# benrobaglia/D2D-PPO

Measured on AMD Instinct MI355X. Metric: env-steps/sec (agents×envs) + PPO updates/sec, 64 agents × 8 ch, 1/2/4/8 GPU, higher is better.
Workload: dtype u8

## Files before the change

### d2d-ppo_amd/csrc/common.h

```cpp
#pragma once
#include <hip/hip_runtime.h>
#include <stdint.h>

#include "d2d_hip.h"

namespace d2d {

constexpr int kWave = 64;

enum : uint32_t { kStreamFlip = 0, kStreamArrival = 1, kStreamAction = 2, kPerEnv = 0xFFFFFFFFu };

struct u32x4 {
  uint32_t x, y, z, w;
};

__device__ __forceinline__ u32x4 philox(uint32_t c0, uint32_t c1, uint32_t c2, uint32_t c3, uint64_t seed) {
  uint32_t k0 = (uint32_t)seed, k1 = (uint32_t)(seed >> 32);
#pragma unroll
  for (int r = 0; r < 10; ++r) {
    if (r) {
      k0 += 0x9E3779B9u;
      k1 += 0xBB67AE85u;
    }
    const uint64_t p0 = (uint64_t)0xD2511F53u * c0;
    const uint64_t p1 = (uint64_t)0xCD9E8D57u * c2;
    uint32_t n0, n2;
    asm("v_bitop3_b32 %0, %1, %2, %3 bitop3:0x96" : "=v"(n0) : "v"((uint32_t)(p1 >> 32)), "v"(c1), "s"(k0));
    asm("v_bitop3_b32 %0, %1, %2, %3 bitop3:0x96" : "=v"(n2) : "v"((uint32_t)(p0 >> 32)), "v"(c3), "s"(k1));
    c0 = n0;
    c1 = (uint32_t)p1;
    c2 = n2;
    c3 = (uint32_t)p0;
  }
  return {c0, c1, c2, c3};
}

__device__ __forceinline__ uint32_t pick(const u32x4& r, int i) {
  return i == 0 ? r.x : (i == 1 ? r.y : (i == 2 ? r.z : r.w));
}

__device__ __forceinline__ uint32_t poisson_lookup(uint32_t r, const uint32_t* __restrict__ t) {
  uint32_t x = 0;
  for (;;) {
    const uint4 q = *reinterpret_cast<const uint4*>(t + x);
    const uint32_t n = (uint32_t)(r > q.x) + (uint32_t)(r > q.y) + (uint32_t)(r > q.z) + (uint32_t)(r > q.w);
    x += n;
    if (n < 4u) return x;
  }
}

}

void d2d_set_error(const char* fmt, ...);

#define D2D_CHECK_HIP(expr)                                                    \
  do {                                                                         \
    hipError_t _e = (expr);                                                    \
    if (_e != hipSuccess) {                                                    \
      d2d_set_error("%s: %s", #expr, hipGetErrorString(_e));                   \
      return D2D_EHIP;                                                         \
    }                                                                          \
  } while (0)

inline int obs_format_args(int32_t format, const uint32_t* sgn_in, int32_t obs_dim, const void* obs, const float*& f32,
                           const uint8_t*& rec, const uint32_t*& sgn) {
  f32 = nullptr; rec = nullptr; sgn = nullptr;
  if (format == D2D_OBS_F32) { f32 = static_cast<const float*>(obs); return D2D_OK; }
  if (format != D2D_OBS_U8) { d2d_set_error("unknown obs_format %d", format); return D2D_EINVAL; }
  if (!sgn_in) { d2d_set_error("obs_format D2D_OBS_U8 needs obs_signed"); return D2D_EINVAL; }
  if (reinterpret_cast<uintptr_t>(obs) & 15) { d2d_set_error("the obs record must be 16-byte aligned"); return D2D_EINVAL; }
  (void)obs_dim;
  rec = static_cast<const uint8_t*>(obs); sgn = sgn_in;
  return D2D_OK;
}
```

### d2d-ppo_amd/csrc/env_kernels.hip

```cpp
#include <atomic>
#include <cmath>
#include <cstdarg>
#include <cstdio>
#include <cstring>

#include "common.h"
#include "policy_split.h"

namespace d2d {

constexpr int kBlock = 256;
constexpr int kCombWavesPerEu = 7;
constexpr int kCombRecBlock = 256;
constexpr int kMaxAgents = 1024;

struct EnvArgs {
  int E, N, C, D, F, S, state_stride, seg, reset, cnt_words;
  uint32_t flags;
  uint32_t rng_step;
  uint64_t env_base, seed;
  const d2d_agent_entry* agents;
  const uint64_t* flip_thr;
  const uint32_t* pois_cdf;
  uint32_t* buf;
  void* chan;
  uint32_t* recv;
  uint32_t* disc;
  uint32_t* selq;
  uint32_t* seln;
  const void* actions;
  const void* flips;
  const uint8_t* arrivals;
  float* obs;
  uint8_t* rec;
  int rec_bytes;
  float* state;
  uint16_t* state_b;
  int64_t state_b_ld;
  int32_t* reward;
  void* ack;
  uint8_t* success;
  const int32_t* gather;
  const uint32_t* rng_off;
  uint64_t draw[kMaxAgents / 64];
};

template <int DW>
struct Row {
  uint32_t w[DW];
};

template <int DW>
__device__ __forceinline__ void load_row(Row<DW>& r, const uint32_t* p) {
  if constexpr (DW == 4) {
    const uint4 v = *reinterpret_cast<const uint4*>(p);
    r.w[0] = v.x; r.w[1] = v.y; r.w[2] = v.z; r.w[3] = v.w;
  } else if constexpr (DW == 2) {
    const uint2 v = *reinterpret_cast<const uint2*>(p);
    r.w[0] = v.x; r.w[1] = v.y;
  } else if constexpr (DW == 8) {
    const uint4 v0 = reinterpret_cast<const uint4*>(p)[0];
    const uint4 v1 = reinterpret_cast<const uint4*>(p)[1];
    r.w[0] = v0.x; r.w[1] = v0.y; r.w[2] = v0.z; r.w[3] = v0.w;
    r.w[4] = v1.x; r.w[5] = v1.y; r.w[6] = v1.z; r.w[7] = v1.w;
  } else {
#pragma unroll
    for (int i = 0; i < DW; ++i) r.w[i] = p[i];
  }
}

template <int DW>
__device__ __forceinline__ void store_row(const Row<DW>& r, uint32_t* p) {
  if constexpr (DW == 4) {
    *reinterpret_cast<uint4*>(p) = make_uint4(r.w[0], r.w[1], r.w[2], r.w[3]);
  } else if constexpr (DW == 2) {
    *reinterpret_cast<uint2*>(p) = make_uint2(r.w[0], r.w[1]);
  } else if constexpr (DW == 8) {
    reinterpret_cast<uint4*>(p)[0] = make_uint4(r.w[0], r.w[1], r.w[2], r.w[3]);
    reinterpret_cast<uint4*>(p)[1] = make_uint4(r.w[4], r.w[5], r.w[6], r.w[7]);
  } else {
#pragma unroll
    for (int i = 0; i < DW; ++i) p[i] = r.w[i];
  }
}

template <int DW>
__device__ __forceinline__ bool row_any(const Row<DW>& r) {
// ... 66 lines not shown

template <typename T>
__device__ __forceinline__ void st_stream(T* p, const T& v, bool nt) {
  if (nt)
    __builtin_nontemporal_store(v, p);
  else
    *p = v;
}

__device__ __forceinline__ void flush_contig(float* __restrict__ dst, const float* src, int count, bool nt) {
  const bool vec = ((reinterpret_cast<uintptr_t>(dst) & 15) == 0) && ((count & 3) == 0);
  if (vec) {
    float4* d4 = reinterpret_cast<float4*>(dst);
    const float4* s4 = reinterpret_cast<const float4*>(src);
    for (int i = threadIdx.x; i < (count >> 2); i += blockDim.x) {
      const float4 v = s4[i];
      if (nt) {
        __builtin_nontemporal_store(v.x, &d4[i].x);
        __builtin_nontemporal_store(v.y, &d4[i].y);
        __builtin_nontemporal_store(v.z, &d4[i].z);
        __builtin_nontemporal_store(v.w, &d4[i].w);
      } else {
        d4[i] = v;
      }
    }
  } else {
    for (int i = threadIdx.x; i < count; i += blockDim.x) st_stream(dst + i, src[i], nt);
  }
}

__device__ __forceinline__ void flush_rows(float* __restrict__ dst, int stride, const float* src, int rows, int S,
                                           bool nt) {
  if ((S & 3) == 0 && (stride & 3) == 0 && ((reinterpret_cast<uintptr_t>(dst) & 15) == 0)) {
    const int q = S >> 2;
    for (int i = threadIdx.x; i < rows * q; i += blockDim.x) {
      const int r = i / q, j = i - r * q;
      float4* d4 = reinterpret_cast<float4*>(dst + (size_t)r * stride) + j;
      const float4 v = reinterpret_cast<const float4*>(src + r * S)[j];
      if (nt) {
        __builtin_nontemporal_store(v.x, &d4->x);
        __builtin_nontemporal_store(v.y, &d4->y);
        __builtin_nontemporal_store(v.z, &d4->z);
        __builtin_nontemporal_store(v.w, &d4->w);
      } else {
        *d4 = v;
      }
    }
  } else {
    for (int i = threadIdx.x; i < rows * S; i += blockDim.x) {
      const int r = i / S, j = i - r * S;
      st_stream(dst + (size_t)r * stride + j, src[r * S + j], nt);
    }
  }
}

struct Lane {
  int env, k, local_env, envs_per_block, lane;
  bool active;
  uint64_t segmask;
};

template <bool LARGE>
__device__ __forceinline__ Lane lane_geometry(const EnvArgs& a, int bidx = blockIdx.x) {
  Lane L;
  L.lane = threadIdx.x & (kWave - 1);
  if (LARGE) {
    L.env = bidx;
    L.k = threadIdx.x;
    L.local_env = 0;
    L.envs_per_block = 1;
    L.segmask = ~0ull;
  } else {
    L.local_env = threadIdx.x / a.seg;
    L.k = threadIdx.x - L.local_env * a.seg;
    L.envs_per_block = blockDim.x / a.seg;
    L.env = bidx * L.envs_per_block + L.local_env;
    const int seg_base = L.lane & ~(a.seg - 1);
    L.segmask = (a.seg == kWave) ? ~0ull : (((1ull << a.seg) - 1ull) << seg_base);
  }
  L.active = (L.k < a.N) && (L.env < a.E);
  return L;
}

template <bool LARGE>
__device__ __forceinline__ int env_count(bool v, const Lane& L, int* lds_acc) {
  const int part = __popcll(__ballot(v) & L.segmask);
  if (!LARGE) return part;
  if (L.lane == 0) atomicAdd(lds_acc, part);
  __syncthreads();
  const int tot = *lds_acc;
  return tot;
}

__device__ __forceinline__ void wave_lds_sync() {
  __builtin_amdgcn_s_waitcnt(0xC07F);
  __builtin_amdgcn_wave_barrier();
  asm volatile("" ::: "memory");
}

__device__ __forceinline__ void wave_flush(float* __restrict__ dst, const float* src, int count, bool nt) {
  const int lane = threadIdx.x & (kWave - 1);
  if (((reinterpret_cast<uintptr_t>(dst) & 15) == 0) && ((reinterpret_cast<uintptr_t>(src) & 15) == 0) &&
      ((count & 3) == 0)) {
    float4* d4 = reinterpret_cast<float4*>(dst);
    const float4* s4 = reinterpret_cast<const float4*>(src);
    for (int i = lane; i < (count >> 2); i += kWave) {
      const float4 v = s4[i];
      if (nt) {
        __builtin_nontemporal_store(v.x, &d4[i].x);
        __builtin_nontemporal_store(v.y, &d4[i].y);
        __builtin_nontemporal_store(v.z, &d4[i].z);
        __builtin_nontemporal_store(v.w, &d4[i].w);
      } else {
        d4[i] = v;
      }
    }
  } else {
    for (int i = lane; i < count; i += kWave) st_stream(dst + i, src[i], nt);
  }
}

__device__ __forceinline__ void flush_bf16(uint16_t* __restrict__ dst, const float* src, int S, int first, int stride,
                                           bool nt) {
  const int q8 = (S + 7) >> 3;
  for (int q = first; q < q8; q += stride) {
    uint32_t w[4];
#pragma unroll
    for (int p = 0; p < 4; ++p) {
      const int j = 8 * q + 2 * p;
      const uint32_t lo = j < S ? __float_as_uint(src[j]) >> 16 : 0u;
      const uint32_t hi = j + 1 < S ? __float_as_uint(src[j + 1]) & 0xFFFF0000u : 0u;
      w[p] = lo | hi;
    }
    st_rec(reinterpret_cast<uint4*>(dst) + q, w[0], w[1], w[2], w[3], nt);
  }
}

template <typename MaskT, int DW, bool LARGE, int CT, bool RESET, bool PACKED = false>
__device__ __forceinline__ void comb_step(const EnvArgs a, float* lds, int bidx, uint4* lrec, int lstride, int lenv0) {
  const Lane L = lane_geometry<LARGE>(a, bidx);
  const int N = a.N, F = a.F;
  const int C = CT ? CT : a.C;
  const int wave = threadIdx.x >> 6;
  const int nwaves = blockDim.x >> 6;
  int* cnt = reinterpret_cast<int*>(lds);
  const int slot = (kWave * F + 3) & ~3;
  float* lds_obs = lds + a.cnt_words + wave * slot;
  const int epw = LARGE ? 1 : kWave / a.seg;
  float* lds_state = LARGE ? lds + a.cnt_words + nwaves * slot
                           : lds + a.cnt_words + nwaves * slot + wave * ((epw * a.S + 3) & ~3);
  const size_t row = (size_t)L.env * N + L.k;
  const uint64_t genv = a.env_base + (uint64_t)L.env;
  const uint32_t cmask = (C >= 32) ? 0xFFFFFFFFu : ((1u << C) - 1u);
  constexpr int kMaskShift = 32 - 8 * (int)sizeof(MaskT);
  constexpr uint32_t kRowKeep = sizeof(MaskT) >= 4 ? 0u : ((1u << (kMaskShift & 31)) - 1u);

  Row<DW> b;
#pragma unroll
  for (int i = 0; i < DW; ++i) b.w[i] = 0;
  uint32_t h_pre = cmask, act = 0, rc = 0, dc = 0;
  d2d_agent_entry ag{};
  if (L.active) {
    ag = a.agents[L.k];
    if (!RESET) {
      load_row<DW>(b, a.buf + row * DW);
      act = (uint32_t)reinterpret_cast<const MaskT*>(a.actions)[row] & cmask;
      if constexpr (PACKED) {
        h_pre = (b.w[DW - 1] >> kMaskShift) & cmask;
        b.w[DW - 1] &= kRowKeep;
        const uint32_t cw = a.recv[row];
        rc = cw & 0xFFFFu;
        dc = cw >> 16;
      } else {
        h_pre = (uint32_t)reinterpret_cast<const MaskT*>(a.chan)[row] & cmask;
        rc = a.recv[row];
        dc = a.disc[row];
      }
    }
  }
  if (LARGE) {
    if (threadIdx.x < 80) cnt[threadIdx.x] = 0;
    __syncthreads();
  }

  uint32_t ack_one = cmask, ack_zero = 0, h_new = h_pre;
  bool succ = false;
  int nsucc = 0;
  if (!RESET) {
    ack_one = 0;
    const uint32_t att = row_any<DW>(b) ? act : 0u;
    const uint32_t good = att & h_pre;
    auto count_channel = [&](int c) {
      const uint64_t m = __ballot((att >> c) & 1u) & L.segmask;
      const uint64_t g = __ballot((good >> c) & 1u) & L.segmask;
      if (!LARGE) {
        const int n = __popcll(m);
        ack_zero |= (uint32_t)(n == 0) << c;
        ack_one |= (uint32_t)(n == 1 && g != 0) << c;
      } else if (L.lane == 0) {
        atomicAdd(&cnt[c], __popcll(m));
        atomicAdd(&cnt[32 + c], __popcll(g));
      }
    };
    if constexpr (CT != 0) {
#pragma unroll
      for (int c = 0; c < CT; ++c) count_channel(c);
    } else {
      for (int c = 0; c < C; ++c) count_channel(c);
    }
    if (LARGE) {
      __syncthreads();
      for (int c = 0; c < C; ++c) {
        const int n = cnt[c];
        ack_zero |= (uint32_t)(n == 0) << c;
        ack_one |= (uint32_t)(n == 1 && cnt[32 + c] == 1) << c;
      }
    }
    succ = L.active && ((good & ack_one) != 0);
    nsucc = env_count<LARGE>(succ, L, cnt + 64);
    if (succ) row_remove_first<DW>(b);
    dc += row_expire_shift<DW>(b);
    uint32_t f = 0;
    if (L.active) {
      if (a.flips) {
        f = (uint32_t)reinterpret_cast<const MaskT*>(a.flips)[row];
      } else {
        const uint64_t* thr = a.flip_thr + (size_t)L.k * C;
        auto flip_block = [&](int blk) {
          const u32x4 r = philox((uint32_t)genv, (uint32_t)L.k, rng_of(a), (kStreamFlip << 24) | (uint32_t)blk, a.seed);
#pragma unroll
          for (int i = 0; i < 4; ++i) {
            const int c = blk * 4 + i;
            if (c < C) f |= (uint32_t)((uint64_t)pick(r, i) < thr[c]) << c;
          }
        };
        if constexpr (CT != 0) {
#pragma unroll
          for (int blk = 0; blk < (CT + 3) / 4; ++blk) flip_block(blk);
        } else {
          for (int blk = 0; blk * 4 < C; ++blk) flip_block(blk);
        }
      }
    }
    h_new = (h_pre ^ f) & cmask;
  }
  const bool drew = L.active && (LARGE ? draws_now(a, L.k) : ((a.draw[0] >> L.k) & 1ull));
  if (drew) {
    const uint32_t x = arrival_value(a, ag, row, L.k, genv);
    row_set<DW>(b, (int)ag.deadline - 1, x);
    rc = (RESET ? 0u : rc) + x;
  } else if (RESET) {
    rc = 0;
  }
  if (RESET) dc = 0;
  if (L.active) {
    if constexpr (PACKED) {
      Row<DW> o = b;
      o.w[DW - 1] |= h_new << kMaskShift;
      store_row<DW>(o, a.buf + row * DW);
      a.recv[row] = rc | (dc << 16);
    } else {
      store_row<DW>(b, a.buf + row * DW);
      reinterpret_cast<MaskT*>(a.chan)[row] = (MaskT)h_new;
      a.recv[row] = rc;
      a.disc[row] = dc;
    }
    if (!RESET) {
      if (a.success) a.success[row] = succ ? 1 : 0;
      if (L.k == 0) {
        if (a.reward) a.reward[L.env] = nsucc;
        if (a.ack) {
          int8_t* ak = reinterpret_cast<int8_t*>(a.ack) + (size_t)L.env * C;
          for (int c = 0; c < C; ++c) ak[c] = ((ack_one >> c) & 1) ? 1 : (((ack_zero >> c) & 1) ? 0 : -1);
        }
      }
    }
  }
  const int wave_env0 = LARGE ? bidx : (bidx * L.envs_per_block + wave * epw);
  const int wave_nenv = LARGE ? 1 : max(0, min(epw, a.E - wave_env0));
  if (a.obs) {
    if (L.active) {
      const int lrow = LARGE ? (L.k - wave * kWave) : ((L.local_env - wave * epw) * N + L.k);
      float* o = lds_obs + lrow * F;
      const int w = ag.obs_width;
#pragma unroll
      for (int j = 0; j < DW * 4; ++j)
        if (j < w) o[j] = row_byte<DW>(b, j);
      auto obs_channel = [&](int c) {
        o[w + c] = (float)((h_pre >> c) & 1u);
        o[w + C + c] = ((ack_one >> c) & 1u) ? 1.f : (((ack_zero >> c) & 1u) ? 0.f : -1.f);
      };
      if constexpr (CT != 0) {
#pragma unroll
        for (int c = 0; c < CT; ++c) obs_channel(c);
      } else {
        for (int c = 0; c < C; ++c) obs_channel(c);
      }
      for (int j = w + 2 * C; j < F; ++j) o[j] = 0.f;
    }
    wave_lds_sync();
    if (LARGE) {
      const int k0 = wave * kWave;
      const int nrows = max(0, min(kWave, N - k0));
      if (nrows > 0) wave_flush(a.obs + ((size_t)bidx * N + k0) * F, lds_obs, nrows * F, a.flags & 1u);
    } else if (wave_nenv > 0) {
      wave_flush(a.obs + (size_t)wave_env0 * N * F, lds_obs, wave_nenv * N * F, a.flags & 1u);
    }
  }
  if (a.rec && L.active) {
    const int w = ag.obs_width;
    const uint32_t ack_neg = ~(ack_one | ack_zero) & cmask;
    auto tail_byte = [&](int p) -> uint32_t {
      const int m = p - w;
      if (m < C) return (h_pre >> m) & 1u;
      const int c = m - C;
      if (c < C) return ((ack_one >> c) & 1u) | (((ack_neg >> c) & 1u) * 0xFFu);
      return p == F ? 1u : 0u;
    };
    uint4* dst = reinterpret_cast<uint4*>(a.rec + row * (size_t)a.rec_bytes);
    uint32_t v[8];
    bool built = false;
    if constexpr (CT != 0 && 2 * CT <= 16 && 4 * DW <= 16) {
      if (a.rec_bytes == 32) {
        constexpr int NB = CT / 2;
        auto expand4 = [](uint32_t n) { return (n * 0x204081u) & 0x01010101u; };
        uint32_t blk[NB];
#pragma unroll
        for (int u = 0; u < CT / 4; ++u) {
          blk[u] = expand4((h_pre >> (4 * u)) & 0xFu);
          blk[CT / 4 + u] = expand4((ack_one >> (4 * u)) & 0xFu) | expand4((ack_neg >> (4 * u)) & 0xFu) * 0xFFu;
        }
        const int ws = w >> 2, bs = w & 3;
        uint32_t sh[NB + 1];
#pragma unroll
        for (int j = 0; j <= NB; ++j) {
          const uint32_t hi = j < NB ? blk[j] : 0u, lo = j > 0 ? blk[j - 1] : 0u;
          sh[j] = bs == 0 ? hi : __builtin_amdgcn_alignbyte(hi, lo, 4 - bs);
        }
#pragma unroll
        for (int q = 0; q < 8; ++q) {
          uint32_t word = q < DW ? b.w[q < DW ? q : 0] : 0u;
#pragma unroll
          for (int c = 0; c <= 16 / 4; ++c)
            if (q - c >= 0 && q - c <= NB) word |= ws == c ? sh[q - c] : 0u;
          word |= (q == (F >> 2)) ? (1u << (8 * (F & 3))) : 0u;
          v[q] = word;
        }
        const bool nt = a.flags & 1u;
        st_rec(dst, v[0], v[1], v[2], v[3], nt);
        st_rec(dst + 1, v[4], v[5], v[6], v[7], nt);
        if (lrec) {
          uint4* l = lrec + (size_t)L.k * lstride + 2 * (L.env - lenv0);
          l[0] = make_uint4(v[0], v[1], v[2], v[3]);
          l[1] = make_uint4(v[4], v[5], v[6], v[7]);
        }
        built = true;
      }
    }
    if (!built) {
#pragma unroll
    for (int q = 0; q < 8; ++q) {
      uint32_t word = 0;
#pragma unroll
      for (int j = 0; j < 4; ++j) {
        const int p = 4 * q + j;
        const uint32_t bb = p < 4 * DW ? (b.w[(p < 4 * DW ? p : 0) >> 2] >> (8 * (p & 3))) & 0xFFu : 0u;
        word |= (p < w ? bb : tail_byte(p)) << (8 * j);
      }
      v[q] = word;
    }
    dst[0] = make_uint4(v[0], v[1], v[2], v[3]);
    dst[1] = make_uint4(v[4], v[5], v[6], v[7]);
    if (lrec) {
      uint4* l = lrec + (size_t)L.k * lstride + 2 * (L.env - lenv0);
      l[0] = make_uint4(v[0], v[1], v[2], v[3]);
      l[1] = make_uint4(v[4], v[5], v[6], v[7]);
    }
    for (int q32 = 1; q32 < a.rec_bytes / 32; ++q32) {
#pragma unroll
      for (int q = 0; q < 8; ++q) {
        uint32_t word = 0;
#pragma unroll
        for (int j = 0; j < 4; ++j) word |= tail_byte(32 * q32 + 4 * q + j) << (8 * j);
        v[q] = word;
      }
      dst[2 * q32] = make_uint4(v[0], v[1], v[2], v[3]);
      dst[2 * q32 + 1] = make_uint4(v[4], v[5], v[6], v[7]);
    }
    }
  }
  if (a.state || a.state_b) {
    if (L.active) {
      float* st = lds_state + (LARGE ? 0 : (L.local_env - wave * epw) * a.S);
      const int off = ag.state_offset, d = ag.deadline;
#pragma unroll
      for (int j = 0; j < DW * 4; ++j)
        if (j < d) st[off + j] = row_byte<DW>(b, j);
      const int sb = a.S - C * (N + 1);
      for (int c = 0; c < C; ++c) st[sb + L.k * C + c] = (float)((h_new >> c) & 1u);
      if (L.k == 0)
        for (int c = 0; c < C; ++c)
          st[sb + N * C + c] = ((ack_one >> c) & 1u) ? 1.f : (((ack_zero >> c) & 1u) ? 0.f : -1.f);
    }
    if (LARGE) {
      __syncthreads();
      if (a.state) flush_rows(a.state + (size_t)bidx * a.state_stride, a.state_stride, lds_state, 1, a.S, a.flags & 1u);
      if (a.state_b) flush_bf16(a.state_b + (size_t)bidx * a.state_b_ld, lds_state, a.S, threadIdx.x, blockDim.x, a.flags & 1u);
    } else {
      wave_lds_sync();
      for (int r = 0; r < wave_nenv; ++r) {
        if (a.state)
          wave_flush(a.state + (size_t)(wave_env0 + r) * a.state_stride, lds_state + r * a.S, a.S, a.flags & 1u);
        if (a.state_b)
          flush_bf16(a.state_b + (size_t)(wave_env0 + r) * a.state_b_ld, lds_state + r * a.S, a.S, L.lane, kWave,
                     a.flags & 1u);
      }
    }
  }
}

template <typename MaskT, int DW, bool LARGE, int CT, bool RESET, bool PACKED = false>
__global__ __launch_bounds__(kMaxAgents) __attribute__((amdgpu_waves_per_eu(kCombWavesPerEu))) void comb_kernel(EnvArgs a) {
  extern __shared__ __attribute__((aligned(16))) float lds[];
  comb_step<MaskT, DW, LARGE, CT, RESET, PACKED>(a, lds, blockIdx.x, nullptr, 0, 0);
}

template <int DW, bool PACK>
__global__ __launch_bounds__(256) void comb_state_repack_kernel(int64_t n, uint32_t* buf, uint8_t* chan, uint32_t* recv,
                                                                uint32_t* disc, uint32_t* rows, uint32_t* counters) {
  const int64_t i = (int64_t)blockIdx.x * blockDim.x + threadIdx.x;
  if (i >= n) return;
  Row<DW> b;
  if (PACK) {
    load_row<DW>(b, buf + i * DW);
    b.w[DW - 1] = (b.w[DW - 1] & 0x00FFFFFFu) | ((uint32_t)chan[i] << 24);
    store_row<DW>(b, rows + i * DW);
    counters[i] = (recv[i] & 0xFFFFu) | (disc[i] << 16);
  } else {
    load_row<DW>(b, rows + i * DW);
    chan[i] = (uint8_t)(b.w[DW - 1] >> 24);
    b.w[DW - 1] &= 0x00FFFFFFu;
    store_row<DW>(b, buf + i * DW);
    const uint32_t cw = counters[i];
    recv[i] = cw & 0xFFFFu;
    disc[i] = cw >> 16;
  }
}

template <int DW, int HT, int SE, int MODE>
__global__ __launch_bounds__(256, SE <= 32 ? 2 : 1) void comb_policy_fused_kernel(EnvArgs e, MlpArgs p) {
  static_assert(SE % 32 == 0, "the policy runs 16-env tiles in pairs");
  constexpr int LSTR = 2 * SE + 1;
  __shared__ uint4 lrec[64 * LSTR];
  const int env0 = blockIdx.x * SE;
  for (int q = 0; q < SE / 4; ++q)
    comb_step<uint8_t, DW, false, 8, false>(e, nullptr, blockIdx.x * (SE / 4) + q, lrec, LSTR, env0);
  __syncthreads();
  const uint32_t rng = (MODE == kModeSample && p.rng_off) ? p.rng_step + *p.rng_off : p.rng_step;
  const int lane = threadIdx.x & 63, g = lane >> 4, i = lane & 15;
  const int wave = __builtin_amdgcn_readfirstlane(threadIdx.x >> 6);
  for (int k = wave; k < p.N; k += 4) {
    SplitNet<1, HT, true, false> net;
    net.load(p, k, g, i);
    uint32_t sm[1][2];
    record_sign_masks<1>(sm, p.sgn, k, g);
    const uint4* row = lrec + k * LSTR;
    auto tile = [&](int t, f32x4& lg) {
      const uint2 w = reinterpret_cast<const uint2*>(row + 2 * (16 * t + i))[g];
      const uint32_t d[1][2] = {{w.x, w.y}};
      float xc[1][8];
      stage_record_words<1>(xc, d, sm);
      float v;
      net.template tile<true>(xc, lg, v);
    };
    for (int tt = 0; tt < SE / 16; tt += 2) {
      f32x4 lg0, lg1;
      tile(tt, lg0);
      tile(tt + 1, lg1);
      f32x4 lgc;
#pragma unroll
      for (int r = 0; r < 4; ++r) lgc[r] = uf(__builtin_amdgcn_permlane32_swap(fu(lg0[r]), fu(lg1[r]), false, false)[0]);
      const int envc = env0 + tt * 16 + i + (g < 2 ? 0 : 16);
      policy_epilogue<0, false, true, MODE>(p, lgc, 0.f, envc, envc < p.E, k, g, rng);
    }
  }
}

template <int DW, bool LARGE>
__global__ __launch_bounds__(kMaxAgents) void chsel_kernel(EnvArgs a) {
  extern __shared__ __attribute__((aligned(16))) float lds[];
  const Lane L = lane_geometry<LARGE>(a);
  const int N = a.N, C = a.C, F = a.F;
  int* cnt_all = reinterpret_cast<int*>(lds);
  int* cnt = cnt_all + L.local_env * 34;
  float* lds_obs = lds + a.cnt_words;
  float* lds_state = lds_obs + ((L.envs_per_block * N * F + 3) & ~3);
  const size_t row = (size_t)L.env * N + L.k;
  const uint64_t genv = a.env_base + (uint64_t)L.env;
  const uint32_t hmask = (C + 1 >= 32) ? 0xFFFFFFFFu : ((1u << (C + 1)) - 1u);
  uint32_t* chan = reinterpret_cast<uint32_t*>(a.chan);
  const bool env_ok = L.env < a.E;

  Row<DW> b;
#pragma unroll
  for (int i = 0; i < DW; ++i) b.w[i] = 0;
  uint32_t H = hmask, act = 0, rc = 0, dc = 0;
  d2d_agent_entry ag{};
// ... 341 lines not shown
  if (!comb && !single && d->env_kind != D2D_ENV_CHANNEL_SELECTION) { d2d_set_error("unknown env_kind %d", d->env_kind); return D2D_EINVAL; }
  if (single) {
    if (d->n_agents < 1 || d->n_agents > kMaxAgents) { d2d_set_error("n_agents=%d outside [1,%d]", d->n_agents, kMaxAgents); return D2D_EUNSUPPORTED; }
    if (d->n_channels != 1) { d2d_set_error("the single-channel env needs n_channels == 1"); return D2D_EINVAL; }
    if (d->max_deadline < 1 || d->max_deadline > 32) { d2d_set_error("max_deadline=%d outside [1,32]", d->max_deadline); return D2D_EUNSUPPORTED; }
    if (d->n_envs < 0) { d2d_set_error("n_envs < 0"); return D2D_EINVAL; }
    if (d->obs_dim < 2 || d->state_dim != 0 && d->state_stride < d->state_dim) { d2d_set_error("bad obs/state dims"); return D2D_EINVAL; }
    if (!d->agents || !d->flip_thr || !d->arrival_kind_host || !d->period_host || !d->offset_host || !d->gather ||
        !d->poisson_cdf) {
      d2d_set_error("desc tables (incl. the gather map and poisson_cdf) must be non-NULL"); return D2D_EINVAL;
    }
    return D2D_OK;
  }
  if (d->n_agents < 1 || d->n_agents > kMaxAgents) { d2d_set_error("n_agents=%d outside [1,%d]", d->n_agents, kMaxAgents); return D2D_EUNSUPPORTED; }
  if (d->n_channels < 1 || d->n_channels > (comb ? 32 : 31)) { d2d_set_error("n_channels=%d unsupported", d->n_channels); return D2D_EUNSUPPORTED; }
  if (d->max_deadline < 1 || d->max_deadline > 32) { d2d_set_error("max_deadline=%d outside [1,32]", d->max_deadline); return D2D_EUNSUPPORTED; }
  if (d->n_envs < 0) { d2d_set_error("n_envs < 0"); return D2D_EINVAL; }
  const int F = comb ? d->max_deadline + 2 * d->n_channels : d->max_deadline + d->n_channels + 1;
  if (d->obs_dim != F) { d2d_set_error("obs_dim=%d, expected %d", d->obs_dim, F); return D2D_EINVAL; }
  if (d->state_stride < d->state_dim) { d2d_set_error("state_stride < state_dim"); return D2D_EINVAL; }
  if (!d->agents || !d->flip_thr || !d->arrival_kind_host || !d->period_host || !d->offset_host || !d->poisson_cdf) {
    d2d_set_error("desc tables (incl. poisson_cdf) must be non-NULL"); return D2D_EINVAL;
  }
  return D2D_OK;
}

void draw_mask(const d2d_env_desc* d, int t, uint64_t* mask) {
  memset(mask, 0, sizeof(uint64_t) * (kMaxAgents / 64));
  for (int k = 0; k < d->n_agents; ++k) {
    const int kind = d->arrival_kind_host[k];
    bool dr = kind == D2D_ARRIVAL_POISSON;
    if (kind == D2D_ARRIVAL_SCHEDULED_BERNOULLI) dr = std::fmod((double)t, d->period_host[k]) == d->offset_host[k];
    if (dr) mask[k >> 6] |= 1ull << (k & 63);
  }
}

template <typename K>
int set_lds(K kernel, size_t bytes) {
  if (bytes > 163840) { d2d_set_error("LDS requirement %zu B exceeds 160 KiB (N*obs_dim too large)", bytes); return D2D_EUNSUPPORTED; }
  if (bytes > 65536)
    D2D_CHECK_HIP(hipFuncSetAttribute(reinterpret_cast<const void*>(kernel), hipFuncAttributeMaxDynamicSharedMemorySize, (int)bytes));
  return D2D_OK;
}

size_t lds_need(const EnvArgs& a, int block, int kind) {
  const bool large = a.N > kWave;
  const bool stage = a.obs || a.state || a.state_b;
  const bool comb = kind == D2D_ENV_COMBINATORIAL;
  if (kind == D2D_ENV_SINGLE) {
    const int epb = large ? 1 : block / a.seg;
    return sizeof(float) * ((size_t)a.cnt_words + (size_t)epb * a.N * (a.D <= 4 ? 2 : a.D <= 8 ? 3 : a.D <= 12 ? 4 : a.D <= 16 ? 5 : 9) +
                            (a.rec ? (size_t)a.N * (a.rec_bytes + 4) : 0));
  }
  if (comb) {
    const int nwaves = block / kWave;
    const int epw = large ? 1 : kWave / a.seg;
    const size_t slot = (size_t)((kWave * a.F + 3) & ~3);
    size_t w = (size_t)a.cnt_words + (stage ? nwaves * slot : 0);
    if (a.state || a.state_b) w += large ? (size_t)a.S : (size_t)nwaves * ((epw * a.S + 3) & ~3);
    return sizeof(float) * w;
  }
  const int epb = large ? 1 : block / a.seg;
  return sizeof(float) * ((size_t)a.cnt_words + (size_t)(stage ? ((epb * a.N * a.F + 3) & ~3) : 0) +
                          (a.state ? (size_t)epb * a.S : 0));
}

template <typename K>
int launch(K kernel, const EnvArgs& a, int block, hipStream_t s, int kind) {
  const bool large = a.N > kWave;
  const int epb = large ? 1 : block / a.seg;
  const int grid = (a.E + epb - 1) / epb;
  if (grid == 0) return D2D_OK;
  const size_t lds = lds_need(a, block, kind);
  int rc = set_lds(kernel, lds);
  if (rc) return rc;
  hipLaunchKernelGGL(kernel, dim3(grid), dim3(block), lds, s, a);
  D2D_CHECK_HIP(hipGetLastError());
  return D2D_OK;
}

template <typename MaskT, int DW, int CT, bool RESET, bool PACKED = false>
int dispatch_comb_ct(const EnvArgs& a, int block, hipStream_t s) {
  if (a.N > kWave) return launch(comb_kernel<MaskT, DW, true, CT, RESET, PACKED>, a, block, s, D2D_ENV_COMBINATORIAL);
  return launch(comb_kernel<MaskT, DW, false, CT, RESET, PACKED>, a, block, s, D2D_ENV_COMBINATORIAL);
}

template <int DW>
int dispatch_comb_packed(const EnvArgs& a, int block, hipStream_t s) {
  if (a.reset) return dispatch_comb_ct<uint8_t, DW, 0, true, true>(a, block, s);
  if (a.C == 8) return dispatch_comb_ct<uint8_t, DW, 8, false, true>(a, block, s);
  if (a.C == 4) return dispatch_comb_ct<uint8_t, DW, 4, false, true>(a, block, s);
  return dispatch_comb_ct<uint8_t, DW, 0, false, true>(a, block, s);
}

template <int DW>
int dispatch_comb(const EnvArgs& a, int block, hipStream_t s, bool packed) {
  if (packed) return dispatch_comb_packed<DW>(a, block, s);
  const int C = a.C;
  if (a.reset) {
    if (C <= 8) return dispatch_comb_ct<uint8_t, DW, 0, true>(a, block, s);
    if (C <= 16) return dispatch_comb_ct<uint16_t, DW, 0, true>(a, block, s);
    return dispatch_comb_ct<uint32_t, DW, 0, true>(a, block, s);
  }
  if (C == 8) return dispatch_comb_ct<uint8_t, DW, 8, false>(a, block, s);
  if (C == 4) return dispatch_comb_ct<uint8_t, DW, 4, false>(a, block, s);
  if (C == 16) return dispatch_comb_ct<uint16_t, DW, 16, false>(a, block, s);
  if (C <= 8) return dispatch_comb_ct<uint8_t, DW, 0, false>(a, block, s);
  if (C <= 16) return dispatch_comb_ct<uint16_t, DW, 0, false>(a, block, s);
  return dispatch_comb_ct<uint32_t, DW, 0, false>(a, block, s);
}

template <int DW>
int dispatch_dw(const EnvArgs& a, int block, int kind, hipStream_t s, bool packed) {
  if (kind == D2D_ENV_SINGLE) {
    if (a.N > kWave) return launch(single_kernel<DW, true>, a, block, s, kind);
    return launch(single_kernel<DW, false>, a, block, s, kind);
  }
  if (kind == D2D_ENV_CHANNEL_SELECTION) {
    if (a.N > kWave) return launch(chsel_kernel<DW, true>, a, block, s, kind);
    return launch(chsel_kernel<DW, false>, a, block, s, kind);
  }
  return dispatch_comb<DW>(a, block, s, packed);
}

int packed_eligible(const d2d_env_desc* d) {
  if (d->env_kind != D2D_ENV_COMBINATORIAL) {
    d2d_set_error("the packed state exists for the combinatorial env only"); return D2D_EUNSUPPORTED;
  }
  if (d->n_channels > 8) {
    d2d_set_error("the packed state is built for n_channels <= 8 (uint8 masks), got %d", d->n_channels); return D2D_EUNSUPPORTED;
  }
  if (d->max_deadline + 1 > 4 * buffer_words(d->max_deadline)) {
    d2d_set_error("the packed state needs max_deadline + mask bytes <= 4 * buffer words: max_deadline=%d fills its %d-byte row",
                  d->max_deadline, 4 * buffer_words(d->max_deadline));
    return D2D_EUNSUPPORTED;
  }
  return D2D_OK;
}

int env_args(const d2d_env_desc* d, const d2d_env_state* st, const d2d_env_packed_state* pst, bool packed,
             const void* actions, const d2d_env_replay* rp, const d2d_env_out* out, int reset, int t, uint32_t rng_step,
             EnvArgs& a) {
  int rc = check_desc(d);
  if (rc) return rc;
  const bool comb = d->env_kind == D2D_ENV_COMBINATORIAL;
  if (packed) {
    if (!pst || !pst->rows || !pst->counters) { d2d_set_error("packed state buffers must be non-NULL"); return D2D_EINVAL; }
    if ((rc = packed_eligible(d))) return rc;
  } else {
    if (!st || !st->buffers || !st->channels || !st->received || !st->discarded) {
      d2d_set_error("state buffers must be non-NULL"); return D2D_EINVAL;
    }
    if (!comb && (!st->sel_quality || !st->sel_count)) {
      d2d_set_error("chsel / single need sel_quality / sel_count"); return D2D_EINVAL;
    }
  }
  if (!reset && !actions) { d2d_set_error("actions is NULL"); return D2D_EINVAL; }
  memset(&a, 0, sizeof(a));
  a.E = d->n_envs; a.N = d->n_agents; a.C = d->n_channels; a.D = d->max_deadline; a.F = d->obs_dim;
  a.S = d->state_dim; a.state_stride = d->state_stride; a.reset = reset; a.rng_step = rng_step;
  a.env_base = d->env_base; a.seed = d->seed; a.agents = d->agents; a.flip_thr = d->flip_thr;
  a.pois_cdf = d->poisson_cdf;
  if (packed) {
    a.buf = pst->rows; a.recv = pst->counters;
  } else {
    a.buf = st->buffers; a.chan = st->channels; a.recv = st->received; a.disc = st->discarded;
// ... 286 lines not shown
```

Measured before the change: 1.003 billion.

## Add wave-per-env comb step path with scalarized indexing and shared Philox head

Adds a specialized comb_step variant for the case of one environment per 64-lane wave (seg == 64, uint8 masks, non-reset). Env index and ack masks are made wave-uniform through readfirstlane, so address math and masks can live in scalar registers. The Philox rounds that are the same for every stream of a lane are computed once and reused for the flip and arrival draws. Record placement uses a compile-time shift when all lanes share the same offset. This cuts VALU work and RNG cost per step, at the price of more template instantiations and code size.

```diff
diff --git a/d2d-ppo_amd/csrc/common.h b/d2d-ppo_amd/csrc/common.h
--- a/d2d-ppo_amd/csrc/common.h
+++ b/d2d-ppo_amd/csrc/common.h
@@ -22,6 +22,68 @@
       k0 += 0x9E3779B9u;
       k1 += 0xBB67AE85u;
     }
+    const uint64_t p0 = (uint64_t)0xD2511F53u * c0;
+    const uint64_t p1 = (uint64_t)0xCD9E8D57u * c2;
+    uint32_t n0, n2;
+    asm("v_bitop3_b32 %0, %1, %2, %3 bitop3:0x96" : "=v"(n0) : "v"((uint32_t)(p1 >> 32)), "v"(c1), "s"(k0));
+    asm("v_bitop3_b32 %0, %1, %2, %3 bitop3:0x96" : "=v"(n2) : "v"((uint32_t)(p0 >> 32)), "v"(c3), "s"(k1));
+    c0 = n0;
+    c1 = (uint32_t)p1;
+    c2 = n2;
+    c3 = (uint32_t)p0;
+  }
+  return {c0, c1, c2, c3};
+}
+
+struct philox_head {
+  uint32_t y1;
+  uint32_t hi0;
+  uint32_t z3;
+  uint32_t r1hi, r1lo;
+};
+
+__device__ __forceinline__ philox_head philox_head_of(uint32_t c0, uint32_t c1, uint32_t c2, uint64_t seed) {
+  const uint32_t k0 = (uint32_t)seed, k1 = (uint32_t)(seed >> 32);
+  const uint64_t p0 = (uint64_t)0xD2511F53u * c0;
+  const uint64_t p1 = (uint64_t)0xCD9E8D57u * c2;
+  const uint32_t x0 = c1 ^ ((uint32_t)(p1 >> 32) ^ k0);
+  const uint64_t q0 = (uint64_t)0xD2511F53u * x0;
+  const uint32_t z2 = (uint32_t)(q0 >> 32) ^ ((uint32_t)p0 ^ (k1 + 0xBB67AE85u));
+  const uint64_t r1 = (uint64_t)0xCD9E8D57u * z2;
+  return {(uint32_t)p1, (uint32_t)(p0 >> 32), (uint32_t)q0, (uint32_t)(r1 >> 32), (uint32_t)r1};
+}
+
+__device__ __forceinline__ u32x4 philox_tail(const philox_head& h, uint32_t w3, uint64_t seed) {
+  uint32_t k0 = (uint32_t)seed, k1 = (uint32_t)(seed >> 32);
+  const uint32_t c2_1 = h.hi0 ^ w3 ^ k1;
+  k0 += 0x9E3779B9u;
+  k1 += 0xBB67AE85u;
+  const uint64_t q1 = (uint64_t)0xCD9E8D57u * c2_1;
+  const uint32_t c0_2 = (uint32_t)(q1 >> 32) ^ h.y1 ^ k0;
+  k0 += 0x9E3779B9u;
+  k1 += 0xBB67AE85u;
+  const uint64_t r0 = (uint64_t)0xD2511F53u * c0_2;
+  uint32_t c0 = h.r1hi ^ ((uint32_t)q1 ^ k0);
+  uint32_t c1 = h.r1lo;
+  uint32_t c2 = h.z3 ^ ((uint32_t)(r0 >> 32) ^ k1);
+  uint32_t c3u = (uint32_t)r0;
+  k0 += 0x9E3779B9u;
+  k1 += 0xBB67AE85u;
+  uint32_t c3;
+  {
+    const uint64_t p0 = (uint64_t)0xD2511F53u * c0;
+    const uint64_t p1 = (uint64_t)0xCD9E8D57u * c2;
+    uint32_t n0;
+    asm("v_bitop3_b32 %0, %1, %2, %3 bitop3:0x96" : "=v"(n0) : "v"((uint32_t)(p1 >> 32)), "v"(c1), "s"(k0));
+    c0 = n0;
+    c1 = (uint32_t)p1;
+    c2 = (uint32_t)(p0 >> 32) ^ (c3u ^ k1);
+    c3 = (uint32_t)p0;
+  }
+#pragma unroll
+  for (int r = 4; r < 10; ++r) {
+    k0 += 0x9E3779B9u;
+    k1 += 0xBB67AE85u;
     const uint64_t p0 = (uint64_t)0xD2511F53u * c0;
     const uint64_t p1 = (uint64_t)0xCD9E8D57u * c2;
     uint32_t n0, n2;
diff --git a/d2d-ppo_amd/csrc/env_kernels.hip b/d2d-ppo_amd/csrc/env_kernels.hip
--- a/d2d-ppo_amd/csrc/env_kernels.hip
+++ b/d2d-ppo_amd/csrc/env_kernels.hip
@@ -3,6 +3,7 @@
 #include <cstdarg>
 #include <cstdio>
 #include <cstring>
+#include <type_traits>
 
 #include "common.h"
 #include "policy_split.h"
@@ -235,6 +236,18 @@
   return L;
 }
 
+__device__ __forceinline__ Lane wave_geometry(const EnvArgs& a, int bidx) {
+  Lane L;
+  L.lane = threadIdx.x & (kWave - 1);
+  L.k = L.lane;
+  L.envs_per_block = blockDim.x >> 6;
+  L.local_env = __builtin_amdgcn_readfirstlane(threadIdx.x >> 6);
+  L.env = __builtin_amdgcn_readfirstlane(bidx * L.envs_per_block + L.local_env);
+  L.segmask = ~0ull;
+  L.active = L.k < a.N;
+  return L;
+}
+
 template <bool LARGE>
 __device__ __forceinline__ int env_count(bool v, const Lane& L, int* lds_acc) {
   const int part = __popcll(__ballot(v) & L.segmask);
@@ -289,20 +302,27 @@
   }
 }
 
-template <typename MaskT, int DW, bool LARGE, int CT, bool RESET, bool PACKED = false>
+template <typename MaskT, int DW, bool LARGE, int CT, bool RESET, bool PACKED = false, bool WAVE = false>
 __device__ __forceinline__ void comb_step(const EnvArgs a, float* lds, int bidx, uint4* lrec, int lstride, int lenv0) {
-  const Lane L = lane_geometry<LARGE>(a, bidx);
+  static_assert(!WAVE || (!LARGE && !RESET && sizeof(MaskT) == 1), "the wave-per-env path: uint8 masks, N <= 64, the step");
+  const Lane L = WAVE ? wave_geometry(a, bidx) : lane_geometry<LARGE>(a, bidx);
+  if constexpr (WAVE) {
+    if (L.env >= a.E) return;
+  }
   const int N = a.N, F = a.F;
   const int C = CT ? CT : a.C;
-  const int wave = threadIdx.x >> 6;
+  const int wave = WAVE ? L.local_env : (int)(threadIdx.x >> 6);
   const int nwaves = blockDim.x >> 6;
   int* cnt = reinterpret_cast<int*>(lds);
   const int slot = (kWave * F + 3) & ~3;
   float* lds_obs = lds + a.cnt_words + wave * slot;
-  const int epw = LARGE ? 1 : kWave / a.seg;
+  const int epw = (LARGE || WAVE) ? 1 : kWave / a.seg;
   float* lds_state = LARGE ? lds + a.cnt_words + nwaves * slot
                            : lds + a.cnt_words + nwaves * slot + wave * ((epw * a.S + 3) & ~3);
   const size_t row = (size_t)L.env * N + L.k;
+  const size_t row0 = WAVE ? (size_t)L.env * N : row;
+  const uint32_t ko = WAVE ? (uint32_t)L.k : 0u;
+  auto at = [&](auto* base, uint32_t per) { return base + row0 * per + (uint32_t)(ko * per); };
   const uint64_t genv = a.env_base + (uint64_t)L.env;
   const uint32_t cmask = (C >= 32) ? 0xFFFFFFFFu : ((1u << C) - 1u);
   constexpr int kMaskShift = 32 - 8 * (int)sizeof(MaskT);
@@ -313,23 +333,39 @@
   for (int i = 0; i < DW; ++i) b.w[i] = 0;
   uint32_t h_pre = cmask, act = 0, rc = 0, dc = 0;
   d2d_agent_entry ag{};
+  constexpr int kWaveFlipBlocks = 2;
+  philox_head ph{};
+  u32x4 flip_r[kWaveFlipBlocks] = {};
+  uint32_t arr_r = 0;
+  const bool wave_draws = WAVE && !a.arrivals && (a.draw[0] & (N >= kWave ? ~0ull : ((1ull << N) - 1ull))) != 0;
+  auto wave_philox = [&]() {
+    if (a.flips && !wave_draws) return;
+    ph = philox_head_of((uint32_t)genv, (uint32_t)L.k, rng_of(a), a.seed);
+    if (!a.flips) {
+#pragma unroll
+      for (int blk = 0; blk < kWaveFlipBlocks; ++blk)
+        if (blk * 4 < C) flip_r[blk] = philox_tail(ph, (kStreamFlip << 24) | (uint32_t)blk, a.seed);
+    }
+    if (wave_draws) arr_r = philox_tail(ph, kStreamArrival << 24, a.seed).x;
+  };
   if (L.active) {
     ag = a.agents[L.k];
     if (!RESET) {
-      load_row<DW>(b, a.buf + row * DW);
-      act = (uint32_t)reinterpret_cast<const MaskT*>(a.actions)[row] & cmask;
+      load_row<DW>(b, at(a.buf, DW));
+      act = (uint32_t)*at(reinterpret_cast<const MaskT*>(a.actions), 1) & cmask;
       if constexpr (PACKED) {
         h_pre = (b.w[DW - 1] >> kMaskShift) & cmask;
         b.w[DW - 1] &= kRowKeep;
-        const uint32_t cw = a.recv[row];
+        const uint32_t cw = *at(a.recv, 1);
         rc = cw & 0xFFFFu;
         dc = cw >> 16;
       } else {
-        h_pre = (uint32_t)reinterpret_cast<const MaskT*>(a.chan)[row] & cmask;
-        rc = a.recv[row];
-        dc = a.disc[row];
-      }
-    }
+        h_pre = (uint32_t)*at(reinterpret_cast<const MaskT*>(a.chan), 1) & cmask;
+        rc = *at(a.recv, 1);
+        dc = *at(a.disc, 1);
+      }
+    }
+    if constexpr (WAVE) wave_philox();
   }
   if (LARGE) {
     if (threadIdx.x < 80) cnt[threadIdx.x] = 0;
@@ -361,6 +397,10 @@
     } else {
       for (int c = 0; c < C; ++c) count_channel(c);
     }
+    if constexpr (WAVE) {
+      ack_one = __builtin_amdgcn_readfirstlane(ack_one);
+      ack_zero = __builtin_amdgcn_readfirstlane(ack_zero);
+    }
     if (LARGE) {
       __syncthreads();
       for (int c = 0; c < C; ++c) {
@@ -376,7 +416,17 @@
     uint32_t f = 0;
     if (L.active) {
       if (a.flips) {
-        f = (uint32_t)reinterpret_cast<const MaskT*>(a.flips)[row];
+        f = (uint32_t)*at(reinterpret_cast<const MaskT*>(a.flips), 1);
+      } else if constexpr (WAVE) {
+        const uint64_t* thr = a.flip_thr + (uint32_t)(L.k * C);
+#pragma unroll
+        for (int blk = 0; blk < kWaveFlipBlocks; ++blk) {
+#pragma unroll
+          for (int i = 0; i < 4; ++i) {
+            const int c = blk * 4 + i;
+            if (c < C) f |= (uint32_t)((uint64_t)pick(flip_r[blk], i) < thr[c]) << c;
+          }
+        }
       } else {
         const uint64_t* thr = a.flip_thr + (size_t)L.k * C;
         auto flip_block = [&](int blk) {
@@ -399,7 +449,14 @@
   }
   const bool drew = L.active && (LARGE ? draws_now(a, L.k) : ((a.draw[0] >> L.k) & 1ull));
   if (drew) {
-    const uint32_t x = arrival_value(a, ag, row, L.k, genv);
+    uint32_t x;
+    if constexpr (WAVE) {
+      if (a.arrivals) x = *at(a.arrivals, 1);
+      else if (ag.arrival_kind == D2D_ARRIVAL_POISSON) x = poisson_lookup(arr_r, a.pois_cdf + (uint32_t)(L.k * 256));
+      else x = (uint64_t)arr_r < ag.arrival_thr ? 1u : 0u;
+    } else {
+      x = arrival_value(a, ag, row, L.k, genv);
+    }
     row_set<DW>(b, (int)ag.deadline - 1, x);
     rc = (RESET ? 0u : rc) + x;
   } else if (RESET) {
@@ -410,16 +467,16 @@
     if constexpr (PACKED) {
       Row<DW> o = b;
       o.w[DW - 1] |= h_new << kMaskShift;
-      store_row<DW>(o, a.buf + row * DW);
-      a.recv[row] = rc | (dc << 16);
+      store_row<DW>(o, at(a.buf, DW));
+      *at(a.recv, 1) = rc | (dc << 16);
     } else {
-      store_row<DW>(b, a.buf + row * DW);
-      reinterpret_cast<MaskT*>(a.chan)[row] = (MaskT)h_new;
-      a.recv[row] = rc;
-      a.disc[row] = dc;
+      store_row<DW>(b, at(a.buf, DW));
+      *at(reinterpret_cast<MaskT*>(a.chan), 1) = (MaskT)h_new;
+      *at(a.recv, 1) = rc;
+      *at(a.disc, 1) = dc;
     }
     if (!RESET) {
-      if (a.success) a.success[row] = succ ? 1 : 0;
+      if (a.success) *at(a.success, 1) = succ ? 1 : 0;
       if (L.k == 0) {
         if (a.reward) a.reward[L.env] = nsucc;
         if (a.ack) {
@@ -470,7 +527,7 @@
       if (c < C) return ((ack_one >> c) & 1u) | (((ack_neg >> c) & 1u) * 0xFFu);
       return p == F ? 1u : 0u;
     };
-    uint4* dst = reinterpret_cast<uint4*>(a.rec + row * (size_t)a.rec_bytes);
+    uint4* dst = reinterpret_cast<uint4*>(at(a.rec, (uint32_t)a.rec_bytes));
     uint32_t v[8];
     bool built = false;
     if constexpr (CT != 0 && 2 * CT <= 16 && 4 * DW <= 16) {
@@ -483,29 +540,67 @@
           blk[u] = expand4((h_pre >> (4 * u)) & 0xFu);
           blk[CT / 4 + u] = expand4((ack_one >> (4 * u)) & 0xFu) | expand4((ack_neg >> (4 * u)) & 0xFu) * 0xFFu;
         }
-        const int ws = w >> 2, bs = w & 3;
-        uint32_t sh[NB + 1];
-#pragma unroll
-        for (int j = 0; j <= NB; ++j) {
-          const uint32_t hi = j < NB ? blk[j] : 0u, lo = j > 0 ? blk[j - 1] : 0u;
-          sh[j] = bs == 0 ? hi : __builtin_amdgcn_alignbyte(hi, lo, 4 - bs);
+        const bool nt = a.flags & 1u;
+        bool placed = false;
+        if constexpr (WAVE) {
+          const int w0 = __builtin_amdgcn_readfirstlane(w);
+          if (__ballot(w != w0) == 0) {
+            const int ws = w0 >> 2, bs = w0 & 3;
+            uint32_t sh[NB + 1];
+#pragma unroll
+            for (int j = 0; j <= NB; ++j) {
+              const uint32_t hi = j < NB ? blk[j] : 0u, lo = j > 0 ? blk[j - 1] : 0u;
+              if (j > CT / 4)
+                sh[j] = (uint32_t)((((uint64_t)hi << 32) | lo) >> (32 - 8 * bs));
+              else
+                sh[j] = bs == 0 ? hi : __builtin_amdgcn_alignbyte(hi, lo, 4 - bs);
+            }
+            auto place = [&](auto shift) {
+              constexpr int c = decltype(shift)::value;
+#pragma unroll
+              for (int q = 0; q < 8; ++q) {
+                uint32_t word = q < DW ? b.w[q < DW ? q : 0] : 0u;
+                if (q - c >= 0 && q - c <= NB) word |= sh[q - c >= 0 && q - c <= NB ? q - c : 0];
+                word |= (q == (F >> 2)) ? (1u << (8 * (F & 3))) : 0u;
+                v[q] = word;
+              }
+              st_rec(dst, v[0], v[1], v[2], v[3], nt);
+              st_rec(dst + 1, v[4], v[5], v[6], v[7], nt);
+            };
+            switch (ws) {
+              case 0: place(std::integral_constant<int, 0>{}); break;
+              case 1: place(std::integral_constant<int, 1>{}); break;
+              case 2: place(std::integral_constant<int, 2>{}); break;
+              case 3: place(std::integral_constant<int, 3>{}); break;
+              default: place(std::integral_constant<int, 4>{}); break;
+            }
+            placed = true;
+          }
         }
-#pragma unroll
-        for (int q = 0; q < 8; ++q) {
-          uint32_t word = q < DW ? b.w[q < DW ? q : 0] : 0u;
-#pragma unroll
-          for (int c = 0; c <= 16 / 4; ++c)
-            if (q - c >= 0 && q - c <= NB) word |= ws == c ? sh[q - c] : 0u;
-          word |= (q == (F >> 2)) ? (1u << (8 * (F & 3))) : 0u;
-          v[q] = word;
-        }
-        const bool nt = a.flags & 1u;
-        st_rec(dst, v[0], v[1], v[2], v[3], nt);
-        st_rec(dst + 1, v[4], v[5], v[6], v[7], nt);
-        if (lrec) {
-          uint4* l = lrec + (size_t)L.k * lstride + 2 * (L.env - lenv0);
-          l[0] = make_uint4(v[0], v[1], v[2], v[3]);
-          l[1] = make_uint4(v[4], v[5], v[6], v[7]);
+        if (!placed) {
+          const int ws = w >> 2, bs = w & 3;
+          uint32_t sh[NB + 1];
+#pragma unroll
+          for (int j = 0; j <= NB; ++j) {
+            const uint32_t hi = j < NB ? blk[j] : 0u, lo = j > 0 ? blk[j - 1] : 0u;
+            sh[j] = bs == 0 ? hi : __builtin_amdgcn_alignbyte(hi, lo, 4 - bs);
+          }
+#pragma unroll
+          for (int q = 0; q < 8; ++q) {
+            uint32_t word = q < DW ? b.w[q < DW ? q : 0] : 0u;
+#pragma unroll
+            for (int c = 0; c <= 16 / 4; ++c)
+              if (q - c >= 0 && q - c <= NB) word |= ws == c ? sh[q - c] : 0u;
+            word |= (q == (F >> 2)) ? (1u << (8 * (F & 3))) : 0u;
+            v[q] = word;
+          }
+          st_rec(dst, v[0], v[1], v[2], v[3], nt);
+          st_rec(dst + 1, v[4], v[5], v[6], v[7], nt);
+          if (lrec) {
+            uint4* l = lrec + (size_t)L.k * lstride + 2 * (L.env - lenv0);
+            l[0] = make_uint4(v[0], v[1], v[2], v[3]);
+            l[1] = make_uint4(v[4], v[5], v[6], v[7]);
+          }
         }
         built = true;
       }
@@ -572,10 +667,10 @@
   }
 }
 
-template <typename MaskT, int DW, bool LARGE, int CT, bool RESET, bool PACKED = false>
+template <typename MaskT, int DW, bool LARGE, int CT, bool RESET, bool PACKED = false, bool WAVE = false>
 __global__ __launch_bounds__(kMaxAgents) __attribute__((amdgpu_waves_per_eu(kCombWavesPerEu))) void comb_kernel(EnvArgs a) {
   extern __shared__ __attribute__((aligned(16))) float lds[];
-  comb_step<MaskT, DW, LARGE, CT, RESET, PACKED>(a, lds, blockIdx.x, nullptr, 0, 0);
+  comb_step<MaskT, DW, LARGE, CT, RESET, PACKED, WAVE>(a, lds, blockIdx.x, nullptr, 0, 0);
 }
 
 template <int DW, bool PACK>
@@ -1083,6 +1178,9 @@
 template <typename MaskT, int DW, int CT, bool RESET, bool PACKED = false>
 int dispatch_comb_ct(const EnvArgs& a, int block, hipStream_t s) {
   if (a.N > kWave) return launch(comb_kernel<MaskT, DW, true, CT, RESET, PACKED>, a, block, s, D2D_ENV_COMBINATORIAL);
+  if constexpr (!RESET && sizeof(MaskT) == 1) {
+    if (a.seg == kWave) return launch(comb_kernel<MaskT, DW, false, CT, RESET, PACKED, true>, a, block, s, D2D_ENV_COMBINATORIAL);
+  }
   return launch(comb_kernel<MaskT, DW, false, CT, RESET, PACKED>, a, block, s, D2D_ENV_COMBINATORIAL);
 }
 
```

Measured after the change: 1.125 billion, median of 6. +12.2%, better.
